# GuyTevet/motion-diffusion-model

Hardware: NVIDIA H100
Metric: motions/sec (higher is better)
Workload: dtype fp16 operands / fp32 accumulate (in/out projections hi-lo split)

## Files before the change

### motion-diffusion-model_b200/csrc/epilogues.cuh

```cuda
#pragma once
#include <cuda_fp16.h>

#include "gemm.cuh"
#include "ptx.cuh"

namespace b200 {

__device__ __forceinline__ uint32_t slab_off(int r, int j) { return r * 128 + ((j ^ (r & 7)) << 4); }
__device__ __forceinline__ uint32_t slab64_off(int r, int j) { return r * 64 + ((j ^ ((r >> 1) & 3)) << 4); }

__device__ __forceinline__ void split_hi_lo8(const float (&v)[8], uint32_t (&hi)[4], uint32_t (&lo)[4]) {
#pragma unroll
  for (int i = 0; i < 4; ++i) {
    const __half2 h = __floats2half2_rn(v[2 * i], v[2 * i + 1]);
    const float2 f = __half22float2(h);
    const __half2 l = __floats2half2_rn(v[2 * i] - f.x, v[2 * i + 1] - f.y);
    hi[i] = *reinterpret_cast<const uint32_t*>(&h);
    lo[i] = *reinterpret_cast<const uint32_t*>(&l);
  }
}
__device__ __forceinline__ void join_hi_lo8(const uint4& h, const uint4& l, float (&v)[8]) {
  const uint32_t hw[4] = {h.x, h.y, h.z, h.w}, lw[4] = {l.x, l.y, l.z, l.w};
#pragma unroll
  for (int i = 0; i < 4; ++i) {
    const float2 a = __half22float2(*reinterpret_cast<const __half2*>(&hw[i]));
    const float2 b = __half22float2(*reinterpret_cast<const __half2*>(&lw[i]));
    v[2 * i] = a.x + b.x;
    v[2 * i + 1] = a.y + b.y;
  }
}

__device__ __forceinline__ float gelu_erf(float x) {
  const float t = fminf(fabsf(x), 5.5f);
  float q = 1.9175331544829533e-05f;
  q = fmaf(q, t, -0.0006586098461411893f);
  q = fmaf(q, t, 0.007754423655569553f);
  q = fmaf(q, t, -0.05296541005373001f);
  q = fmaf(q, t, -0.4590602517127991f);
  q = fmaf(q, t, -1.1511220932006836f);
  q = fmaf(q, t, -0.9999997019767761f);
  float a;
  asm("ex2.approx.ftz.f32 %0, %1;" : "=f"(a) : "f"(q));
  const float phi = (x >= 0.f) ? (1.0f - a) : (x < -5.5f ? 0.f : a);
  return x * phi;
}

__device__ __forceinline__ void stage_bias(float* bs, const float* bias, int col_base, int N, int lane) {
  __syncwarp();
#pragma unroll
  for (int i = 0; i < 2; ++i) {
    const int idx = i * 128 + lane * 4;
    const int col = col_base + idx;
    float4 v = make_float4(0.f, 0.f, 0.f, 0.f);
    if (col + 3 < N) {
      v = __ldg(reinterpret_cast<const float4*>(bias + col));
    } else {
      if (col + 0 < N) v.x = bias[col + 0];
      if (col + 1 < N) v.y = bias[col + 1];
      if (col + 2 < N) v.z = bias[col + 2];
    }
    *reinterpret_cast<float4*>(bs + idx) = v;
  }
  __syncwarp();
}

__device__ __forceinline__ uint32_t pack_half2(float a, float b) {
  __half2 h = __floats2half2_rn(a, b);
  return *reinterpret_cast<uint32_t*>(&h);
}

template <bool GELU>
struct EpiBiasF16 {
  static constexpr int NSLAB = 1;
  static constexpr int SMEM_PER_WARP = NSLAB * 4096;
  struct Params {
    const float* bias;
  };
  static __device__ __forceinline__ void preload(const Params& p, float* dst, int N, int tid, int nthreads) {
    for (int i = tid; i < N; i += nthreads) dst[i] = p.bias[i];
  }
  static __device__ __forceinline__ void tile_begin(EpiCtx&, const Params&, int, int) {}
  static __device__ __forceinline__ void chunk(EpiCtx& ctx, const Params&, uint32_t (&raw)[32], int row0, int col0, int) {
    chunk_bias(ctx, ctx.bias_all + col0, raw, row0, col0);
  }
  static __device__ __forceinline__ void chunk_bias(EpiCtx& ctx, const float* bs, uint32_t (&raw)[32], int row0, int col0) {
    const int half = (col0 >> 5) & 1;
    uint8_t* slab = ctx.smem + (ctx.seq % NSLAB) * 4096;
    if (half == 0) {
      if (ctx.lane == 0) bulk_wait_group_read<NSLAB - 1>();
      __syncwarp();
    }
    uint32_t pk[16];
#pragma unroll
    for (int j = 0; j < 32; j += 4) {
      const float4 b = *reinterpret_cast<const float4*>(bs + j);
      float x0 = __uint_as_float(raw[j + 0]) + b.x, x1 = __uint_as_float(raw[j + 1]) + b.y;
      float x2 = __uint_as_float(raw[j + 2]) + b.z, x3 = __uint_as_float(raw[j + 3]) + b.w;
      if (GELU) {
        x0 = gelu_erf(x0); x1 = gelu_erf(x1); x2 = gelu_erf(x2); x3 = gelu_erf(x3);
      }
      pk[j / 2] = pack_half2(x0, x1);
      pk[j / 2 + 1] = pack_half2(x2, x3);
    }
#pragma unroll
    for (int j = 0; j < 4; ++j)
      *reinterpret_cast<uint4*>(slab + slab_off(ctx.lane, half * 4 + j)) =
          make_uint4(pk[4 * j], pk[4 * j + 1], pk[4 * j + 2], pk[4 * j + 3]);
    if (half == 1 || col0 + 32 >= ctx.N) {
      fence_proxy_async_smem();
      __syncwarp();
      if (ctx.lane == 0) {
        tma_store_2d(ctx.map_c, slab, col0 - 32 * half, row0);
        bulk_commit_group();
      }
      ctx.seq++;
    }
  }
  static __device__ __forceinline__ void tile_end(EpiCtx&, const Params&, int, int) {}
  static __device__ __forceinline__ void finish(EpiCtx& ctx) {
    if (ctx.lane == 0) bulk_wait_group<0>();
    __syncwarp();
  }
};

struct EpiBiasF16Global : EpiBiasF16<false> {
  static constexpr bool UNSTAGED = true;
  static __device__ __forceinline__ void preload(const Params&, float*, int, int, int) {}
  static __device__ __forceinline__ void chunk(EpiCtx& ctx, const Params& p, uint32_t (&raw)[32], int row0, int col0, int) {
    chunk_bias(ctx, p.bias + col0, raw, row0, col0);
  }
};

template <bool GELU>
struct EpiBiasF16Wide {
  static constexpr int SMEM_PER_WARP = 2 * 4096;
  struct Params {
    const float* bias;
    int lo_col;
  };
  static __device__ __forceinline__ void preload(const Params& p, float* dst, int N, int tid, int nthreads) {
    for (int i = tid; i < N; i += nthreads) dst[i] = p.bias[i];
  }
  static __device__ __forceinline__ void tile_begin(EpiCtx&, const Params&, int, int) {}
  static __device__ __forceinline__ void chunk(EpiCtx& ctx, const Params& p, uint32_t (&raw)[32], int row0, int col0,
                                               int) {
    const int half = (col0 >> 5) & 1;
    uint8_t* slab_hi = ctx.smem;
    uint8_t* slab_lo = ctx.smem + 4096;
    if (half == 0) {
      if (ctx.lane == 0) bulk_wait_group_read<0>();
      __syncwarp();
    }
    const float* bs = ctx.bias_all + col0;
#pragma unroll
    for (int j = 0; j < 4; ++j) {
      uint32_t hi[4], lo[4];
#pragma unroll
      for (int i = 0; i < 4; ++i) {
        float x0 = __uint_as_float(raw[8 * j + 2 * i]) + bs[8 * j + 2 * i];
        float x1 = __uint_as_float(raw[8 * j + 2 * i + 1]) + bs[8 * j + 2 * i + 1];
        if (GELU) {
          x0 = gelu_erf(x0); x1 = gelu_erf(x1);
        }
        const __half2 h = __floats2half2_rn(x0, x1);
        const float2 f = __half22float2(h);
        const __half2 l = __floats2half2_rn(x0 - f.x, x1 - f.y);
        hi[i] = *reinterpret_cast<const uint32_t*>(&h);
        lo[i] = *reinterpret_cast<const uint32_t*>(&l);
      }
      *reinterpret_cast<uint4*>(slab_hi + slab_off(ctx.lane, half * 4 + j)) = make_uint4(hi[0], hi[1], hi[2], hi[3]);
      *reinterpret_cast<uint4*>(slab_lo + slab_off(ctx.lane, half * 4 + j)) = make_uint4(lo[0], lo[1], lo[2], lo[3]);
    }
    if (half == 1 || col0 + 32 >= ctx.N) {
      fence_proxy_async_smem();
      __syncwarp();
      if (ctx.lane == 0) {
        tma_store_2d(ctx.map_c, slab_hi, col0 - 32 * half, row0);
        tma_store_2d(ctx.map_c, slab_lo, p.lo_col + col0 - 32 * half, row0);
        bulk_commit_group();
      }
      ctx.seq++;
    }
  }
  static __device__ __forceinline__ void tile_end(EpiCtx&, const Params&, int, int) {}
  static __device__ __forceinline__ void finish(EpiCtx& ctx) {
    if (ctx.lane == 0) bulk_wait_group<0>();
    __syncwarp();
  }
};

struct EpiEmbed {
  static constexpr int SMEM_PER_WARP = 2 * 4096;
  template <class P> static __device__ __forceinline__ void preload(const P&, float*, int, int, int) {}
  struct Params {
    CUtensorMap res_c, res_u;
    const float* pe_bias;
    int S, d, halves;
  };
  static __device__ __forceinline__ void tile_begin(EpiCtx&, const Params&, int, int) {}
  static __device__ __forceinline__ void chunk(EpiCtx& ctx, const Params& p, uint32_t (&raw)[32], int row0, int col0,
                                               int) {
    uint8_t* slab = ctx.smem + (ctx.seq & 1) * 4096;
    if (ctx.lane == 0) bulk_wait_group_read<1>();
    __syncwarp();
    const int row = row0 + ctx.lane;
    const int s = (row < ctx.M) ? row % p.S : 0;
    const float* pb = p.pe_bias + static_cast<size_t>(s) * p.d + col0;
#pragma unroll
    for (int j = 0; j < 4; ++j) {
      const float4 a0 = __ldg(reinterpret_cast<const float4*>(pb + 8 * j));
      const float4 a1 = __ldg(reinterpret_cast<const float4*>(pb + 8 * j + 4));
      const float o[8] = {__uint_as_float(raw[8 * j + 0]) + a0.x, __uint_as_float(raw[8 * j + 1]) + a0.y,
                          __uint_as_float(raw[8 * j + 2]) + a0.z, __uint_as_float(raw[8 * j + 3]) + a0.w,
                          __uint_as_float(raw[8 * j + 4]) + a1.x, __uint_as_float(raw[8 * j + 5]) + a1.y,
                          __uint_as_float(raw[8 * j + 6]) + a1.z, __uint_as_float(raw[8 * j + 7]) + a1.w};
      uint32_t hi[4], lo[4];
      split_hi_lo8(o, hi, lo);
      *reinterpret_cast<uint4*>(slab + slab64_off(ctx.lane, j)) = make_uint4(hi[0], hi[1], hi[2], hi[3]);
      *reinterpret_cast<uint4*>(slab + 2048 + slab64_off(ctx.lane, j)) = make_uint4(lo[0], lo[1], lo[2], lo[3]);
    }
    fence_proxy_async_smem();
    __syncwarp();
    if (ctx.lane == 0) {
      tma_store_2d(&p.res_c, slab, col0, row0);
      tma_store_2d(&p.res_c, slab + 2048, p.d + col0, row0);
      if (p.halves == 2) {
        tma_store_2d(&p.res_u, slab, col0, row0);
        tma_store_2d(&p.res_u, slab + 2048, p.d + col0, row0);
      }
      bulk_commit_group();
    }
    ctx.seq++;
  }
  static __device__ __forceinline__ void tile_end(EpiCtx&, const Params&, int, int) {}
  static __device__ __forceinline__ void finish(EpiCtx& ctx) {
    if (ctx.lane == 0) bulk_wait_group<0>();
    __syncwarp();
  }
};

constexpr int SCHED_STRIDE = 8;
struct StepState {
  int done;
  int cur;
  int start;
  int pad;
  const float* noise;
  long long noise_step_stride;
  unsigned long long seed;
  long long sample_base;
};

struct EpiOutStep {
  static constexpr int SMEM_PER_WARP = 1024;
  template <class P> static __device__ __forceinline__ void preload(const P&, float*, int, int, int) {}
  struct Params {
    const float* bias;
    const float* x_t;
    const float* noise;
    float* x_out;
    float* pred_xstart;
    const unsigned char* inpaint_mask;
    const float* inpaint_motion;
    const float* sched;
    const StepState* state;
    long long noise_batch_stride;
    int B, S, T, J, mode;
    int s_off;
    int clip_denoised;
  };
  static __device__ __forceinline__ void tile_begin(EpiCtx&, const Params&, int, int) {}
  static __device__ __forceinline__ void chunk(EpiCtx& ctx, const Params& p, uint32_t (&raw)[32], int row0, int col0,
                                               int) {
    const int row = row0 + ctx.lane;
    if (row >= ctx.M) return;
    const int b = row / p.S, s = row - b * p.S;
    if (s < p.s_off) return;
    const int t = s - p.s_off;
    float c1 = 0.f, c2 = 0.f, sg = 0.f, sr = 0.f, srm1 = 1.f, sq = 0.f, ce = 0.f;
    const float* nz = nullptr;
    if (p.mode != 0) {
      const StepState st = *p.state;
      const float* row_s = p.sched + static_cast<size_t>(st.cur) * SCHED_STRIDE;
      c1 = row_s[0]; c2 = row_s[1]; sr = row_s[3]; srm1 = row_s[4]; sq = row_s[5]; ce = row_s[6];
      sg = (p.mode == 1) ? row_s[2] : row_s[7];
      nz = (p.noise != nullptr ? p.noise : st.noise + static_cast<long long>(st.done) * st.noise_step_stride) +
           static_cast<long long>(b) * p.noise_batch_stride;
    }
    const size_t base = static_cast<size_t>(b) * p.J * p.T + t;
#pragma unroll
    for (int h = 0; h < 32; h += 16) {
      float xv[16], nv[16];
#pragma unroll
      for (int j = 0; j < 16; ++j) {
        const int col = col0 + h + j;
        xv[j] = (p.mode != 0 && col < p.J) ? p.x_t[base + static_cast<size_t>(col) * p.T] : 0.f;
        nv[j] = (p.mode != 0 && col < p.J) ? nz[static_cast<size_t>(col) * p.T + t] : 0.f;
      }
#pragma unroll
      for (int j = 0; j < 16; ++j) {
        const int col = col0 + h + j;
        if (col < p.J) {
          const size_t idx = base + static_cast<size_t>(col) * p.T;
          float x0 = __uint_as_float(raw[h + j]) + __ldg(p.bias + col);
          if (p.inpaint_mask != nullptr && p.inpaint_mask[idx]) x0 = p.inpaint_motion[idx];
          if (p.clip_denoised) x0 = fminf(fmaxf(x0, -1.f), 1.f);
          if (p.pred_xstart != nullptr) p.pred_xstart[idx] = x0;
          float o = x0;
          if (p.mode == 1) {
            const float mean = __fadd_rn(__fmul_rn(c1, x0), __fmul_rn(c2, xv[j]));
            o = __fadd_rn(mean, __fmul_rn(sg, nv[j]));
          } else if (p.mode == 2) {
            const float eh = __fdiv_rn(__fsub_rn(__fmul_rn(sr, xv[j]), x0), srm1);
            const float mean = __fadd_rn(__fmul_rn(x0, sq), __fmul_rn(ce, eh));
            o = __fadd_rn(mean, __fmul_rn(sg, nv[j]));
          }
          p.x_out[idx] = o;
        }
      }
    }
  }
  static __device__ __forceinline__ void tile_end(EpiCtx&, const Params&, int, int) {}
  static __device__ __forceinline__ void finish(EpiCtx&) {}
};

}
```

### motion-diffusion-model_b200/csrc/gemm.cuh

```cuda
#pragma once
#include "ptx.cuh"

namespace b200 {

constexpr int GEMM_BLOCK_M = 128;
constexpr int GEMM_BLOCK_K = 64;
constexpr int GEMM_EPI_WARPS = 8;
constexpr int GEMM_THREADS = 384;
constexpr int GEMM_BAR_BYTES = 1024;
constexpr int GEMM_BIAS_BYTES = 8192;

constexpr int GEMM_RES_KB_MAX = 8;
constexpr int GEMM_REGS_PRODUCER = 40, GEMM_REGS_CONSUMER = 232;

template <int BLOCK_N>
constexpr int gemm_stage_cols() { return BLOCK_N < 128 ? BLOCK_N : 128; }
template <int BLOCK_N>
constexpr int gemm_stage_ld() { return gemm_stage_cols<BLOCK_N>() + 4; }

template <int BLOCK_N, class Epi, bool RESIDENT = false>
struct GemmSmem {
  static constexpr int A_BYTES = GEMM_BLOCK_M * GEMM_BLOCK_K * 2;
  static constexpr int B_BYTES = BLOCK_N * GEMM_BLOCK_K * 2;
  static constexpr int STAGE_BYTES = A_BYTES + (RESIDENT ? 0 : B_BYTES);
  static constexpr int W_BYTES = RESIDENT ? GEMM_RES_KB_MAX * B_BYTES : 0;
  static constexpr int ACC_BYTES = 2 * 64 * gemm_stage_ld<BLOCK_N>() * 4;
  static constexpr int EPI_BYTES = GEMM_EPI_WARPS * Epi::SMEM_PER_WARP;
  static constexpr int budget = 227 * 1024 - 1024  - W_BYTES - ACC_BYTES - EPI_BYTES - GEMM_BIAS_BYTES - GEMM_BAR_BYTES;
  static constexpr int STAGES = (budget / STAGE_BYTES) > 6 ? 6 : (budget / STAGE_BYTES);
  static constexpr int TOTAL = 1024 + W_BYTES + STAGES * STAGE_BYTES + EPI_BYTES + ACC_BYTES + GEMM_BIAS_BYTES + GEMM_BAR_BYTES;
  static_assert(STAGES >= 2, "not enough shared memory for a pipeline");
  static_assert(Epi::SMEM_PER_WARP % 1024 == 0, "epilogue slabs must keep 1024-byte alignment (128B swizzle)");
  static_assert(B_BYTES % 1024 == 0, "W tiles must keep 1024-byte alignment (128B swizzle)");
};

struct EpiCtx {
  uint8_t* smem;
  const CUtensorMap* map_c;
  const float* bias_all;
  int lane;
  int M, N;
  int col_base;
  int col_end;
  uint32_t seq;
};

template <int BLOCK_N>
__device__ __forceinline__ void stage_acc(float* st, const float (&acc)[BLOCK_N / 2], int c0, int wq, int lane) {
  constexpr int LD = gemm_stage_ld<BLOCK_N>();
  constexpr int NJ = gemm_stage_cols<BLOCK_N>() / 8;
  const int r = 16 * wq + (lane >> 2), c = 2 * (lane & 3);
#pragma unroll
  for (int jj = 0; jj < NJ; ++jj) {
    const int j = c0 / 8 + jj;
    *reinterpret_cast<float2*>(st + r * LD + 8 * jj + c) = make_float2(acc[4 * j], acc[4 * j + 1]);
    *reinterpret_cast<float2*>(st + (r + 8) * LD + 8 * jj + c) = make_float2(acc[4 * j + 2], acc[4 * j + 3]);
  }
}
template <int BLOCK_N>
__device__ __forceinline__ void load_row32(const float* st, int row, int col, uint32_t (&raw)[32]) {
  constexpr int LD = gemm_stage_ld<BLOCK_N>();
  const float4* p = reinterpret_cast<const float4*>(st + row * LD + col);
#pragma unroll
  for (int i = 0; i < 8; ++i) {
    const float4 v = p[i];
    raw[4 * i] = __float_as_uint(v.x); raw[4 * i + 1] = __float_as_uint(v.y);
    raw[4 * i + 2] = __float_as_uint(v.z); raw[4 * i + 3] = __float_as_uint(v.w);
  }
}

template <int BLOCK_N, class Epi, bool RESIDENT = false>
__global__ void __launch_bounds__(GEMM_THREADS, 1)
gemm_f16_wgmma(const __grid_constant__ CUtensorMap map_a, const __grid_constant__ CUtensorMap map_b,
               const __grid_constant__ CUtensorMap map_c, int M, int N, int K,
               const __grid_constant__ typename Epi::Params ep) {
  using SM = GemmSmem<BLOCK_N, Epi, RESIDENT>;
  using MMA = Wgmma<BLOCK_N>;
  constexpr int STAGES = SM::STAGES;
  constexpr int NREG = BLOCK_N / 2;
  static_assert(BLOCK_N % 32 == 0, "epilogue works on 32-column chunks");

  extern __shared__ uint8_t smem_raw[];
  uint8_t* smem = reinterpret_cast<uint8_t*>((reinterpret_cast<uintptr_t>(smem_raw) + 1023) & ~uintptr_t(1023));
  uint8_t* wres = smem;
  uint8_t* tiles = smem + SM::W_BYTES;
  uint8_t* epi_smem = tiles + STAGES * SM::STAGE_BYTES;
  float* acc_stage = reinterpret_cast<float*>(epi_smem + SM::EPI_BYTES);
  float* bias_all = reinterpret_cast<float*>(epi_smem + SM::EPI_BYTES + SM::ACC_BYTES);
  uint64_t* bars = reinterpret_cast<uint64_t*>(epi_smem + SM::EPI_BYTES + SM::ACC_BYTES + GEMM_BIAS_BYTES);
  uint64_t* full_bar = bars;
  uint64_t* empty_bar = bars + STAGES;
  uint64_t* w_full = bars + 2 * STAGES;

  const int warp = threadIdx.x >> 5;
  const int lane = threadIdx.x & 31;
  const int tiles_m = (M + GEMM_BLOCK_M - 1) / GEMM_BLOCK_M;
  const int tiles_n = (N + BLOCK_N - 1) / BLOCK_N;
  const int num_tiles = tiles_m * tiles_n;
  const int num_kb = (K + GEMM_BLOCK_K - 1) / GEMM_BLOCK_K;
  const int res_n = blockIdx.x % tiles_n;
  const int first = RESIDENT ? (blockIdx.x / tiles_n) * tiles_n + res_n : blockIdx.x;
  const int step = RESIDENT ? ((gridDim.x - res_n + tiles_n - 1) / tiles_n) * tiles_n : gridDim.x;

  pdl_launch_dependents();
  Epi::preload(ep, bias_all, N, threadIdx.x, blockDim.x);
  if (threadIdx.x == 0) {
    tma_prefetch_desc(&map_a);
    tma_prefetch_desc(&map_b);
    tma_prefetch_desc(&map_c);
    for (int s = 0; s < STAGES; ++s) {
      mbar_init(&full_bar[s], 1);
      mbar_init(&empty_bar[s], GEMM_EPI_WARPS);
    }
    if (RESIDENT)
      for (int s = 0; s < GEMM_RES_KB_MAX; ++s) mbar_init(&w_full[s], 1);
    fence_barrier_init();
  }
  __syncthreads();
  pdl_wait();

  if (warp < 4) {
    asm volatile("setmaxnreg.dec.sync.aligned.u32 %0;" ::"n"(GEMM_REGS_PRODUCER));
    if (warp == 0 && elect_one()) {
      int stage = 0;
      uint32_t phase = 0;
      bool first_tile = true;
      for (int tile = first; tile < num_tiles; tile += step) {
        const int m_blk = tile / tiles_n, n_blk = tile % tiles_n;
        for (int kb = 0; kb < num_kb; ++kb) {
          if (RESIDENT && first_tile) {
            mbar_expect_tx(&w_full[kb], SM::B_BYTES);
            tma_load_2d(wres + kb * SM::B_BYTES, &map_b, &w_full[kb], kb * GEMM_BLOCK_K, n_blk * BLOCK_N);
          }
          mbar_wait(&empty_bar[stage], phase ^ 1);
          uint8_t* sa = tiles + stage * SM::STAGE_BYTES;
          mbar_expect_tx(&full_bar[stage], SM::STAGE_BYTES);
          tma_load_2d(sa, &map_a, &full_bar[stage], kb * GEMM_BLOCK_K, m_blk * GEMM_BLOCK_M);
          if (!RESIDENT) tma_load_2d(sa + SM::A_BYTES, &map_b, &full_bar[stage], kb * GEMM_BLOCK_K, n_blk * BLOCK_N);
          if (++stage == STAGES) { stage = 0; phase ^= 1; }
        }
        first_tile = false;
      }
    }
  } else {
    asm volatile("setmaxnreg.inc.sync.aligned.u32 %0;" ::"n"(GEMM_REGS_CONSUMER));
    const int wg = (warp >> 2) - 1;
    const int wq = warp & 3;
    const int part = wq >> 1;
    const int rh = 32 * (wq & 1);
    float* st = acc_stage + wg * 64 * gemm_stage_ld<BLOCK_N>();
    EpiCtx ctx;
    ctx.smem = epi_smem + (warp - 4) * Epi::SMEM_PER_WARP;
    ctx.map_c = &map_c;
    ctx.bias_all = bias_all;
    ctx.lane = lane;
    ctx.M = M;
    ctx.N = N;
    ctx.seq = 0;
    int stage = 0;
    uint32_t phase = 0;
    float acc[NREG];
    bool first_tile = true;
    for (int tile = first; tile < num_tiles; tile += step) {
      const int m_blk = tile / tiles_n, n_blk = tile % tiles_n;
      const int col_base = n_blk * BLOCK_N;
      int prev_stage = -1;
      for (int kb = 0; kb < num_kb; ++kb) {
        if (RESIDENT && first_tile) mbar_wait(&w_full[kb], 0);
        mbar_wait(&full_bar[stage], phase);
        const uint32_t sa = smem_u32(tiles + stage * SM::STAGE_BYTES) + wg * 64 * 128;
        const uint32_t sb = RESIDENT ? smem_u32(wres + kb * SM::B_BYTES) : smem_u32(tiles + stage * SM::STAGE_BYTES) + SM::A_BYTES;
        const uint64_t da = wgmma_desc_k_sw128(sa);
        const uint64_t db = wgmma_desc_k_sw128(sb);
        wgmma_fence_acc(acc);
        wgmma_fence();
#pragma unroll
        for (int k = 0; k < GEMM_BLOCK_K / 16; ++k) MMA::mma(acc, da + 2 * k, db + 2 * k, (kb | k) != 0);
        wgmma_commit();
        wgmma_fence_acc(acc);
        wgmma_wait<1>();
        if (prev_stage >= 0 && lane == 0) mbar_arrive(&empty_bar[prev_stage]);
        prev_stage = stage;
        if (++stage == STAGES) { stage = 0; phase ^= 1; }
      }
      wgmma_wait<0>();
      wgmma_fence_acc(acc);
      if (lane == 0) mbar_arrive(&empty_bar[prev_stage]);
      first_tile = false;
      const int row0 = m_blk * GEMM_BLOCK_M + 64 * wg + rh;
      const bool live = row0 < M;
      ctx.col_base = col_base;
      ctx.col_end = col_base + BLOCK_N;
      if (live) Epi::tile_begin(ctx, ep, row0, col_base);
      uint32_t raw[32];
      auto run = [&](int c0, int c, int cn) {
        if (live && col_base + c < N) {
          load_row32<BLOCK_N>(st, rh + lane, c - c0, raw);
          Epi::chunk(ctx, ep, raw, row0, col_base + c, (cn < BLOCK_N && col_base + cn < N) ? col_base + cn : -1);
        }
      };
      constexpr int SC = gemm_stage_cols<BLOCK_N>();
#pragma unroll
      for (int c0 = 0; c0 < BLOCK_N; c0 += SC) {
        named_bar_sync(1 + wg, 128);
        stage_acc<BLOCK_N>(st, acc, c0, wq, lane);
        named_bar_sync(1 + wg, 128);
        const int c = c0 + part * 64;
        if (c < c0 + SC && c < BLOCK_N) {
          const bool two = c + 32 < BLOCK_N;
          const int cnext = c + 128;
          run(c0, c, two ? c + 32 : cnext);
          if (two) run(c0, c + 32, cnext);
        }
      }
      if (live) Epi::tile_end(ctx, ep, row0, col_base);
    }
    Epi::finish(ctx);
  }
}

}
```

Before: 354.3.

## Write GEMM bias epilogue straight from wgmma fragments into swizzled TMA slabs

Measured after the change: 376.7, median of 6. +6.3%, better.

```diff
diff --git a/motion-diffusion-model_b200/csrc/epilogues.cuh b/motion-diffusion-model_b200/csrc/epilogues.cuh
--- a/motion-diffusion-model_b200/csrc/epilogues.cuh
+++ b/motion-diffusion-model_b200/csrc/epilogues.cuh
@@ -79,6 +79,14 @@
   static __device__ __forceinline__ void preload(const Params& p, float* dst, int N, int tid, int nthreads) {
     for (int i = tid; i < N; i += nthreads) dst[i] = p.bias[i];
   }
+  static constexpr bool FRAGMENT = true;
+  static __device__ __forceinline__ uint32_t pack2(float a0, float a1, float2 b) {
+    float x0 = a0 + b.x, x1 = a1 + b.y;
+    if (GELU) {
+      x0 = gelu_erf(x0); x1 = gelu_erf(x1);
+    }
+    return pack_half2(x0, x1);
+  }
   static __device__ __forceinline__ void tile_begin(EpiCtx&, const Params&, int, int) {}
   static __device__ __forceinline__ void chunk(EpiCtx& ctx, const Params&, uint32_t (&raw)[32], int row0, int col0, int) {
     chunk_bias(ctx, ctx.bias_all + col0, raw, row0, col0);
@@ -94,13 +102,8 @@
 #pragma unroll
     for (int j = 0; j < 32; j += 4) {
       const float4 b = *reinterpret_cast<const float4*>(bs + j);
-      float x0 = __uint_as_float(raw[j + 0]) + b.x, x1 = __uint_as_float(raw[j + 1]) + b.y;
-      float x2 = __uint_as_float(raw[j + 2]) + b.z, x3 = __uint_as_float(raw[j + 3]) + b.w;
-      if (GELU) {
-        x0 = gelu_erf(x0); x1 = gelu_erf(x1); x2 = gelu_erf(x2); x3 = gelu_erf(x3);
-      }
-      pk[j / 2] = pack_half2(x0, x1);
-      pk[j / 2 + 1] = pack_half2(x2, x3);
+      pk[j / 2] = pack2(__uint_as_float(raw[j + 0]), __uint_as_float(raw[j + 1]), make_float2(b.x, b.y));
+      pk[j / 2 + 1] = pack2(__uint_as_float(raw[j + 2]), __uint_as_float(raw[j + 3]), make_float2(b.z, b.w));
     }
 #pragma unroll
     for (int j = 0; j < 4; ++j)
@@ -125,6 +128,7 @@
 
 struct EpiBiasF16Global : EpiBiasF16<false> {
   static constexpr bool UNSTAGED = true;
+  static constexpr bool FRAGMENT = false;
   static __device__ __forceinline__ void preload(const Params&, float*, int, int, int) {}
   static __device__ __forceinline__ void chunk(EpiCtx& ctx, const Params& p, uint32_t (&raw)[32], int row0, int col0, int) {
     chunk_bias(ctx, p.bias + col0, raw, row0, col0);
diff --git a/motion-diffusion-model_b200/csrc/gemm.cuh b/motion-diffusion-model_b200/csrc/gemm.cuh
--- a/motion-diffusion-model_b200/csrc/gemm.cuh
+++ b/motion-diffusion-model_b200/csrc/gemm.cuh
@@ -1,4 +1,6 @@
 #pragma once
+#include <type_traits>
+
 #include "ptx.cuh"
 
 namespace b200 {
@@ -18,13 +20,18 @@
 template <int BLOCK_N>
 constexpr int gemm_stage_ld() { return gemm_stage_cols<BLOCK_N>() + 4; }
 
+template <class Epi, class = void> struct epi_fragment : std::false_type {};
+template <class Epi> struct epi_fragment<Epi, std::enable_if_t<Epi::FRAGMENT>> : std::true_type {};
+template <int BLOCK_N, class Epi>
+constexpr bool gemm_direct_epi() { return epi_fragment<Epi>::value && BLOCK_N <= 128 && BLOCK_N % 64 == 0; }
+
 template <int BLOCK_N, class Epi, bool RESIDENT = false>
 struct GemmSmem {
   static constexpr int A_BYTES = GEMM_BLOCK_M * GEMM_BLOCK_K * 2;
   static constexpr int B_BYTES = BLOCK_N * GEMM_BLOCK_K * 2;
   static constexpr int STAGE_BYTES = A_BYTES + (RESIDENT ? 0 : B_BYTES);
   static constexpr int W_BYTES = RESIDENT ? GEMM_RES_KB_MAX * B_BYTES : 0;
-  static constexpr int ACC_BYTES = 2 * 64 * gemm_stage_ld<BLOCK_N>() * 4;
+  static constexpr int ACC_BYTES = gemm_direct_epi<BLOCK_N, Epi>() ? 0 : 2 * 64 * gemm_stage_ld<BLOCK_N>() * 4;
   static constexpr int EPI_BYTES = GEMM_EPI_WARPS * Epi::SMEM_PER_WARP;
   static constexpr int budget = 227 * 1024 - 1024  - W_BYTES - ACC_BYTES - EPI_BYTES - GEMM_BIAS_BYTES - GEMM_BAR_BYTES;
   static constexpr int STAGES = (budget / STAGE_BYTES) > 6 ? 6 : (budget / STAGE_BYTES);
@@ -69,6 +76,30 @@
   }
 }
 
+template <int BLOCK_N, class Epi>
+__device__ __forceinline__ void epi_direct(uint8_t* slab, const float (&acc)[BLOCK_N / 2], const float* bias_all,
+                                           const CUtensorMap* map_c, int wg, int wq, int lane, int row_base,
+                                           int col_base, int M, int N) {
+  if (lane == 0) bulk_wait_group_read<0>();
+  named_bar_sync(1 + wg, 128);
+  const int r = 16 * wq + (lane >> 2), q = lane & 3;
+#pragma unroll
+  for (int j = 0; j < BLOCK_N / 8; ++j) {
+    const float2 b = *reinterpret_cast<const float2*>(bias_all + col_base + 8 * j + 2 * q);
+    uint8_t* p = slab + (j >> 3) * 8192 + (((j & 7) ^ (r & 7)) << 4) + 4 * q;
+    *reinterpret_cast<uint32_t*>(p + r * 128) = Epi::pack2(acc[4 * j], acc[4 * j + 1], b);
+    *reinterpret_cast<uint32_t*>(p + (r + 8) * 128) = Epi::pack2(acc[4 * j + 2], acc[4 * j + 3], b);
+  }
+  fence_proxy_async_smem();
+  named_bar_sync(1 + wg, 128);
+  const int blk = wq >> 1, h = wq & 1;
+  const int row0 = row_base + 32 * h, col0 = col_base + 64 * blk;
+  if (lane == 0 && 64 * blk < BLOCK_N && row0 < M && col0 < N) {
+    tma_store_2d(map_c, slab + blk * 8192 + h * 4096, col0, row0);
+    bulk_commit_group();
+  }
+}
+
 template <int BLOCK_N, class Epi, bool RESIDENT = false>
 __global__ void __launch_bounds__(GEMM_THREADS, 1)
 gemm_f16_wgmma(const __grid_constant__ CUtensorMap map_a, const __grid_constant__ CUtensorMap map_b,
@@ -76,6 +107,9 @@
                const __grid_constant__ typename Epi::Params ep) {
   using SM = GemmSmem<BLOCK_N, Epi, RESIDENT>;
   using MMA = Wgmma<BLOCK_N>;
+  constexpr bool DIRECT = gemm_direct_epi<BLOCK_N, Epi>();
+  static_assert(!DIRECT || (GEMM_EPI_WARPS / 2) * Epi::SMEM_PER_WARP >= (BLOCK_N / 64) * 8192,
+                "direct epilogue: a warpgroup's warp slabs must hold its [64 x BLOCK_N] fp16 output");
   constexpr int STAGES = SM::STAGES;
   constexpr int NREG = BLOCK_N / 2;
   static_assert(BLOCK_N % 32 == 0, "epilogue works on 32-column chunks");
@@ -187,6 +221,11 @@
       wgmma_fence_acc(acc);
       if (lane == 0) mbar_arrive(&empty_bar[prev_stage]);
       first_tile = false;
+      if constexpr (DIRECT) {
+        epi_direct<BLOCK_N, Epi>(epi_smem + wg * (GEMM_EPI_WARPS / 2) * Epi::SMEM_PER_WARP, acc, bias_all, &map_c, wg, wq,
+                                 lane, m_blk * GEMM_BLOCK_M + 64 * wg, col_base, M, N);
+        continue;
+      }
       const int row0 = m_blk * GEMM_BLOCK_M + 64 * wg + rh;
       const bool live = row0 < M;
       ctx.col_base = col_base;
```
